# nurturenature/jepsen-tigerbeetle

Hardware: AMD Instinct MI355X
Metric: histories/sec, 10k-op/64-proc cas-register histories (time-to-verdict ms in extra) (higher is better)
Workload: dtype u64

## Files before the change

jepsen-tigerbeetle_amd/csrc/batch_create.hip:

```cpp
#include "tbc_batch.h"
#include "reach_table.h"

using namespace tbc;

namespace tbc {

uint64_t open_list_entries(const tbc_ops& c, uint64_t op_off, uint64_t n, uint32_t n_events, uint32_t n_slots,
                                  std::vector<uint32_t>& pre, bool branch_lists) {
  const uint64_t worst = std::max<uint64_t>(n, 1) * std::max(1u, n_slots);
  if (n == 0) return 1;
  if ((uint64_t)n_events > 64 * n + 1024) return worst;
  const uint32_t* inv = c.inv_pos + op_off;
  const uint32_t* ret = c.ret_pos + op_off;
  pre.assign((size_t)n_events + 1, 0u);
  for (uint64_t i = 0; i < n; i++) {
    if (ret[i] == TBC_POS_CRASHED) continue;
    if (ret[i] >= n_events || inv[i] > ret[i]) return worst;
    pre[ret[i] + 1] = 1;
  }
  for (uint32_t x = 1; x <= n_events; x++) pre[x] += pre[x - 1];
  uint64_t total = 0;
  const uint8_t* f = c.f + op_off;
  for (uint64_t i = 0; i < n; i++)
    if (ret[i] != TBC_POS_CRASHED && !(branch_lists && f[i] == TBC_F_READ)) total += pre[ret[i]] - pre[inv[i]] + 1;
// ... 327 lines not shown
    H.rec_off = tot.rec_n; tot.rec_n += n + 2ull * H.n_slots;
    H.seg_off = tot.seg_n; tot.seg_n += H.n_slots + 1;
    H.ret_off = H.op_off;
    H.bm_off = tot.bm_n; tot.bm_n += H.n_events / 32 + 1;
    H.frame_off = tot.frame_n; tot.frame_n += std::max<uint64_t>(n, 1) * B->frame_words;
    const uint64_t per_op = B->opts.visited_per_op ? B->opts.visited_per_op : 64;
    uint32_t lg = std::max(10u, ceil_log2(per_op * std::max<uint64_t>(n, 1)));
    while (lg > 10 && (1ull << lg) * KW * 8 > max_bytes) lg--;
    H.tab_log2 = lg;
    H.tab_off = tot.tab_n;
    if (!beam) { tot.tab_n += (1ull << lg) * KW; tot.tab_n = (tot.tab_n + 1) & ~1ull; }
    if (beam) {
      BeamHist& Q = bh[h];
      std::memset(&Q, 0, sizeof Q);
      uint32_t blg = lg;
      while (blg > 10 && ((1ull << blg) * EW * 8 > max_bytes || blg > kBeamMaxTabLog2)) blg--;
      Q.tab_log2 = blg;
      Q.off_off = tot.boff_n; tot.boff_n += n + 2;
      if (B->count_form) {
        const CountHist& ch = (*count_hist)[h];
        Q.cmem_off = tot.bocc_n; tot.bocc_n += ch.words.size();
        Q.n_classes = ch.n_classes; Q.top[0] = ch.top[0]; Q.top[1] = ch.top[1];
      }
      Q.lst_cap = lists_on_device ? 0xFFFFFFF0u : list_caps[h];
      Q.lst_off = tot.blst_n; tot.blst_n += lists_on_device ? 0u : Q.lst_cap;
      Q.stack_off = tot.bstack_n; tot.bstack_n += (1ull << blg);
      Q.tab_off = tot.btab_n; tot.btab_n += (1ull << blg);
    }
  }
  if (B->sweep) { tot.bstack_n = 0; tot.btab_n = 0; }
  return TBC_OK;
}

}

void tbc_batch::count_device_bytes() {
  tbc_batch* const B = this;
  const bool beam = B->width > 1;
  B->device_bytes = B->d_f.bytes() + B->d_a.bytes() + B->d_b.bytes() + B->d_proc.bytes() + B->d_inv.bytes() +
                    B->d_ret.bytes() + B->d_hist.bytes() + B->d_rec.bytes() + B->d_seg.bytes() + B->d_ret_slot.bytes() +
                    B->d_ret_op.bytes() + B->d_bitmap.bytes() + B->d_wpre.bytes() + B->d_frames.bytes() +
                    B->d_tab.bytes() + B->d_results.bytes() + B->d_work.bytes() + B->d_witness.bytes();
  if (beam) B->device_bytes += B->d_bh.bytes() + B->d_off.bytes() + B->d_ncr.bytes() + B->d_lst.bytes() +
                               B->d_crashed.bytes() + B->d_slot8.bytes() + B->d_rk8.bytes() + B->d_twn.bytes() + B->d_rdm.bytes() + B->d_look.bytes() + B->d_looktmp.bytes() + B->d_dstack.bytes() + B->d_stack.bytes() + B->d_btab.bytes() + B->d_pool.bytes() + B->d_cmem.bytes();
  if (B->d_stage[0].p) B->device_bytes += B->d_stage[0].bytes();
  if (B->d_stage[1].p) B->device_bytes += B->d_stage[1].bytes();
}

tbc_batch::~tbc_batch() {
  tbc::stream_release(this);
  d_f.release(); d_a.release(); d_b.release(); d_proc.release(); d_inv.release(); d_ret.release();
  d_hist.release(); d_rec.release(); d_seg.release(); d_ret_slot.release(); d_ret_op.release();
  d_bitmap.release(); d_wpre.release(); d_frames.release(); d_witness.release(); d_work.release();
  d_queue.release(); d_tab.release(); d_results.release(); d_table.release(); d_pool_vals.release(); d_cfg.release();
  d_bh.release(); d_off.release(); d_ncr.release(); d_lst.release(); d_crashed.release(); d_stack.release();
  d_zncr.release(); d_reach.release(); d_reach_hdr.release(); d_abort.release(); d_order.release(); d_park.release();
  if (abort_one) (void)hipHostFree(abort_one);
  if (progress) (void)hipHostFree(progress);
  d_progress.release();
  if (!borrowed) { for (auto& e : ev2) if (e) (void)hipEventDestroy(e); if (stream2) (void)hipStreamDestroy(stream2); }
  d_cmem.release(); d_occ.release(); d_btab.release(); d_slot8.release(); d_rk8.release(); d_look.release(); d_looktmp.release(); d_twn.release(); d_rdm.release(); d_cuts.release(); d_seglist.release(); d_sres.release(); d_dstack.release(); d_pool.release(); d_pool_cursor.release();
  if (ev_turn) (void)hipEventDestroy(ev_turn);
  if (!borrowed) {
    for (auto& e : ev) if (e) (void)hipEventDestroy(e);
    if (stream) (void)hipStreamDestroy(stream);
  }
}

namespace tbc {
namespace {

tbc_status alloc_arenas(CreatePlan& P) {
  tbc_batch* B = P.B; const tbc_opts* opts = P.opts; const tbc_model* model = P.model;
  const uint32_t nh = P.nh;
  const bool beam = P.beam, device_sizing = P.device_sizing;
  const LayoutTotals& t = P.tot;
  const uint32_t EW = B->entry_words();
  tbc_status s;
  const uint64_t T = B->total_ops;
  if (!t_ctx) {
    HIP_TRY(hipHostMalloc((void**)&B->progress, 16 * sizeof(uint32_t), hipHostMallocMapped | hipHostMallocCoherent));
    std::memset(B->progress, 0, 16 * sizeof(uint32_t));
    if ((s = B->d_progress.alloc(1))) return s;
  }
  if ((s = B->d_f.alloc(T)) || (s = B->d_a.alloc(T)) || (s = B->d_b.alloc(T)) || (s = B->d_proc.alloc(T)) ||
      (s = B->d_inv.alloc(T)) || (s = B->d_ret.alloc(T)) || (s = B->d_hist.alloc(nh)) || (s = B->d_bh.alloc(beam ? nh : 0)) || (s = B->d_work.alloc(nh)) ||
      (s = B->d_bitmap.alloc(t.bm_n)) || (s = B->d_off.alloc(beam ? t.boff_n : 0)) || (s = B->d_ncr.alloc(beam ? t.boff_n : 0)) || (s = B->d_pool_cursor.alloc(1)) ||
      (s = B->d_rec.alloc(t.rec_n)) ||
      (s = B->d_seg.alloc(t.seg_n)) || (s = B->d_ret_slot.alloc(T)) || (s = B->d_ret_op.alloc(T)) ||
      (s = B->d_wpre.alloc(t.bm_n)) || (s = B->d_frames.alloc(t.frame_n)) ||
      (s = B->d_tab.alloc(t.tab_n)) || (s = B->d_results.alloc(nh)) ||
      (s = B->d_queue.alloc(4)) || (s = B->d_witness.alloc(opts->want_witness ? T : 0)))
    return s;
  if (beam) {
    if ((!device_sizing && (s = B->d_lst.alloc(t.blst_n))) || (s = B->d_crashed.alloc((B->count_form || !B->any_crashed) ? 0 : T)) || (s = B->d_cmem.alloc(B->count_form ? t.bocc_n : 0)) ||
        (s = B->d_slot8.alloc(slot8_bytes(T, nh))) || (s = B->d_stack.alloc(t.bstack_n)) || (s = B->d_btab.alloc(t.btab_n * B->tab_stride())))
      return s;
    if ((B->sweep || B->rsweep) && ((s = B->d_cuts.alloc((uint64_t)nh * B->max_segs)) || (s = B->d_sres.alloc((uint64_t)nh * B->max_segs * kSweepSlices)) || (s = B->d_seglist.alloc((uint64_t)nh * B->max_segs * kSweepSlices * 3)))) return s;
    if (B->sweep || B->rsweep) B->seg_host.resize((size_t)nh * B->max_segs * kSweepSlices);
    if (B->rsweep) {
      std::vector<uint32_t> reach, hdr;
      for (uint32_t h = 0; h < nh; h++) {
        const CountHist& ch = B->count_hist[h];
        hdr.push_back((uint32_t)reach.size());
        hdr.push_back(build_reach_table(ch.words.data(), ch.n_classes, reach));
      }
      if ((s = B->d_zncr.alloc(t.boff_n)) || (s = B->d_reach.alloc(reach.size())) || (s = B->d_reach_hdr.alloc(hdr.size())) || (s = B->d_abort.alloc(nh))) return s;
      HIP_TRY(hipMemset(B->d_zncr.p, 0, B->d_zncr.bytes()));
      HIP_TRY(hipMemcpy(B->d_reach.p, reach.data(), reach.size() * 4, hipMemcpyHostToDevice));
      HIP_TRY(hipMemcpy(B->d_reach_hdr.p, hdr.data(), hdr.size() * 4, hipMemcpyHostToDevice));
      HIP_TRY(hipHostMalloc((void**)&B->abort_one, sizeof(uint32_t), hipHostMallocDefault));
      *B->abort_one = 1u;
    }
    if (B->lanes && (s = B->d_rk8.alloc(slot8_bytes(T, nh)))) return s;
    if (B->reg_rules() && ((!device_sizing && (s = B->d_twn.alloc(t.blst_n * B->mask_words))) || (s = B->d_rdm.alloc(B->lanes ? 1 : T * B->vpad * B->mask_words)))) return s;
    if (B->lanes) { B->d_rdm.release(); if ((s = B->d_rdm.alloc(T * B->front_words()))) return s; }
    const bool by_front = B->mask_words == 1 && B->vpad <= 32;
    if (B->lookahead && ((s = B->d_look.alloc(look_words(T, nh, B->mask_words))) || (s = B->d_looktmp.alloc(by_front ? 0 : T)) ||
                         (s = B->d_dstack.alloc(t.bstack_n)))) return s;
    {
      uint64_t biggest = 0;
      for (uint32_t h = 0; h < nh; h++) biggest = std::max<uint64_t>(biggest, 1ull << B->bh[h].tab_log2);
      uint64_t words = std::max<uint64_t>(t.btab_n * B->tab_stride() * (B->lanes ? 1u : 3u) / 10, biggest * (4 + 16 + 4) * (EW + 1));
      words = std::min<uint64_t>(words, (32ull << 30) / 8);
      if (B->sweep) words = 1;
      if ((s = B->d_pool.alloc(words))) return s;
    }
  }
  if ((s = B->d_cfg.alloc((uint64_t)nh * kCfgCap * (2 + B->mask_words)))) return s;
  if (beam && (s = B->d_park.alloc((uint64_t)nh * kParkWords))) return s;
  B->pool_len = P.desc->cols.pool ? P.desc->cols.pool_len : 0;
  if ((s = B->d_pool_vals.alloc(B->pool_len))) return s;
  if (B->pool_len) HIP_TRY(hipMemcpy(B->d_pool_vals.p, P.desc->cols.pool, (size_t)B->pool_len * 4, hipMemcpyHostToDevice));
  if (model->kind == TBC_MODEL_TABLE) {
    const size_t tn = (size_t)model->n_states * model->n_classes;
    B->table_host.assign(model->table, model->table + tn);
    if ((s = B->d_table.alloc(tn))) return s;
    HIP_TRY(hipMemcpy(B->d_table.p, B->table_host.data(), tn * 2, hipMemcpyHostToDevice));
    B->model.table = nullptr;
  }
  B->count_device_bytes();
  return TBC_OK;
}

tbc_status take_streams(tbc_batch* B) {
  if (t_ctx) {
    B->borrowed = true; B->stream = t_ctx->stream;
    for (int i = 0; i < 6; i++) B->ev[i] = t_ctx->ev[i];
    if (B->rsweep) {
      if (!t_ctx->stream2) {
        HIP_TRY(hipStreamCreateWithFlags(&t_ctx->stream2, hipStreamNonBlocking));
        for (auto& e : t_ctx->ev2) HIP_TRY(hipEventCreate(&e));
      }
      B->stream2 = t_ctx->stream2; B->ev2[0] = t_ctx->ev2[0]; B->ev2[1] = t_ctx->ev2[1];
    }
  } else {
    HIP_TRY(hipStreamCreateWithFlags(&B->stream, hipStreamNonBlocking));
    for (auto& e : B->ev) HIP_TRY(hipEventCreate(&e));
    if (B->rsweep) {
      HIP_TRY(hipStreamCreateWithFlags(&B->stream2, hipStreamNonBlocking));
      for (auto& e : B->ev2) HIP_TRY(hipEventCreate(&e));
    }
  }
  return TBC_OK;
}

tbc_status upload_inputs(CreatePlan& P, bool* done) {
  tbc_batch* B = P.B; const tbc_batch_desc* desc = P.desc;
  const uint32_t nh = P.nh;
  const bool beam = P.beam, device_sizing = P.device_sizing;
  const uint64_t T = B->total_ops, bocc_n = P.tot.bocc_n;
  *done = false;
  std::vector<uint32_t> work(nh);
  for (uint32_t h = 0; h < nh; h++) work[h] = h;
  if (t_ctx && T && !(B->count_form && bocc_n) && !device_sizing) {
    char* const base = (char*)B->d_f.p;
    const auto at = [&](const void* p) { return (size_t)((const char*)p - base); };
    const auto a256 = [](size_t b) { return (b + 255) & ~(size_t)255; };
    const bool consecutive = !B->d_f.owned && !B->d_a.owned && !B->d_b.owned && !B->d_proc.owned && !B->d_inv.owned && !B->d_ret.owned && !B->d_hist.owned &&
                             !B->d_bh.owned && !B->d_work.owned && at(B->d_a.p) == a256(T) && at(B->d_b.p) == at(B->d_a.p) + a256(T * 4) &&
                             at(B->d_proc.p) == at(B->d_b.p) + a256(T * 4) && at(B->d_inv.p) == at(B->d_proc.p) + a256(T * 4) && at(B->d_ret.p) == at(B->d_inv.p) + a256(T * 4) &&
                             at(B->d_hist.p) == at(B->d_ret.p) + a256(T * 4) && at(B->d_bh.p) == at(B->d_hist.p) + a256(nh * sizeof(Hist)) &&
                             at(B->d_work.p) == at(B->d_bh.p) + a256(std::max<size_t>(beam ? nh : 0, 1) * sizeof(BeamHist));
    if (consecutive) {
      const size_t total = at(B->d_work.p) + a256((size_t)nh * 4);
      B->upload_stage.resize(total);
      if (B->upload_stage.own.empty()) {
        char* st = B->upload_stage.data();
        std::memcpy(st, desc->cols.f, T);
        std::memcpy(st + at(B->d_a.p), desc->cols.a, T * 4);
        std::memcpy(st + at(B->d_b.p), desc->cols.b, T * 4);
        std::memcpy(st + at(B->d_proc.p), B->count_form ? P.slot_col.data() : desc->cols.process, T * 4);
        std::memcpy(st + at(B->d_inv.p), desc->cols.inv_pos, T * 4);
        std::memcpy(st + at(B->d_ret.p), desc->cols.ret_pos, T * 4);
        std::memcpy(st + at(B->d_hist.p), B->hist.data(), nh * sizeof(Hist));
        if (beam) std::memcpy(st + at(B->d_bh.p), B->bh.data(), nh * sizeof(BeamHist));
        std::memcpy(st + at(B->d_work.p), work.data(), (size_t)nh * 4);
        HIP_TRY(hipMemcpyAsync(base, st, total, hipMemcpyHostToDevice, B->stream));
        B->inputs_fresh = true;
        *done = true;
        TRACE("create: inputs queued as one block");
        return TBC_OK;
      }
    }
  }
  if (T) {
    HIP_TRY(hipMemcpyAsync(B->d_f.p, desc->cols.f, T, hipMemcpyHostToDevice, B->stream));
    HIP_TRY(hipMemcpyAsync(B->d_a.p, desc->cols.a, T * 4, hipMemcpyHostToDevice, B->stream));
    HIP_TRY(hipMemcpyAsync(B->d_b.p, desc->cols.b, T * 4, hipMemcpyHostToDevice, B->stream));
    HIP_TRY(hipMemcpyAsync(B->d_proc.p, B->count_form ? P.slot_col.data() : desc->cols.process, T * 4, hipMemcpyHostToDevice, B->stream));
    HIP_TRY(hipMemcpyAsync(B->d_inv.p, desc->cols.inv_pos, T * 4, hipMemcpyHostToDevice, B->stream));
    HIP_TRY(hipMemcpyAsync(B->d_ret.p, desc->cols.ret_pos, T * 4, hipMemcpyHostToDevice, B->stream));
  }
  std::vector<uint64_t> cmem_host;
  if (B->count_form && bocc_n) {
    cmem_host.reserve(bocc_n);
    for (uint32_t h = 0; h < nh; h++) cmem_host.insert(cmem_host.end(), B->count_hist[h].words.begin(), B->count_hist[h].words.end());
    HIP_TRY(hipMemcpyAsync(B->d_cmem.p, cmem_host.data(), cmem_host.size() * 8, hipMemcpyHostToDevice, B->stream));
  }
  HIP_TRY(hipMemcpyAsync(B->d_hist.p, B->hist.data(), nh * sizeof(Hist), hipMemcpyHostToDevice, B->stream));
  HIP_TRY(hipMemcpyAsync(B->d_work.p, work.data(), nh * 4, hipMemcpyHostToDevice, B->stream));
  HIP_TRY(hipStreamSynchronize(B->stream));
  TRACE("create: inputs resident");
  return TBC_OK;
}
// ... 157 lines not shown
```

jepsen-tigerbeetle_amd/csrc/batch_run.hip:

```cpp
#include "tbc_batch.h"
#include "witness_expand.h"

using namespace tbc;

namespace tbc {

static SearchArgs make_search_args(tbc_batch* B, uint64_t* tab, uint32_t n_work) {
  SearchArgs a{};
  a.hist = B->d_hist.p; a.rec = B->d_rec.p; a.seg = B->d_seg.p; a.ret_slot = B->d_ret_slot.p;
  a.ret_op = B->d_ret_op.p;
  a.frames = B->d_frames.p; a.tab = tab; a.results = B->d_results.p;
  a.witness = B->opts.want_witness ? B->d_witness.p : nullptr;
  a.work = B->d_work.p; a.queue = B->d_queue.p;
  a.table = B->d_table.p; a.n_work = n_work; a.model_kind = B->model.kind;
  a.init_state = B->model.init;
  a.n_classes = B->model.n_classes; a.n_states = B->model.n_states;
  a.max_steps = B->opts.max_steps;
  a.time_limit_ticks = B->opts.time_limit_ms * 100000ull;
  a.dbg = debug_words();
  a.pool_vals = B->d_pool_vals.p;
  a.cfg = B->d_cfg.p;
  a.progress = B->progress; a.progress_dev = B->d_progress.p;
  return a;
}

PackArgs make_pack_args(tbc_batch* B) {
  PackArgs pa{};
  pa.hist = B->d_hist.p; pa.f = B->d_f.p; pa.a = B->d_a.p; pa.b = B->d_b.p; pa.process = B->d_proc.p;
  pa.inv_pos = B->d_inv.p; pa.ret_pos = B->d_ret.p; pa.rec = B->d_rec.p; pa.seg = B->d_seg.p;
  pa.ret_slot = B->d_ret_slot.p; pa.ret_op = B->d_ret_op.p; pa.bitmap = B->d_bitmap.p; pa.wpre = B->d_wpre.p;
  pa.scratch = B->d_frames.p; pa.frame_words = B->frame_words; pa.n_hist = B->n_hist;
  pa.model_kind = B->model.kind; pa.n_classes = B->model.n_classes; pa.dbg = debug_words();
  pa.pool_vals = B->d_pool_vals.p; pa.pool_len = B->pool_len; pa.n_keys = B->model.n_keys;
  return pa;
}

PackOpenArgs make_pack_open_args(tbc_batch* B) {
  PackOpenArgs po{};
  po.hist = B->d_hist.p; po.bh = B->d_bh.p; po.f = B->d_f.p; po.a = B->d_a.p; po.b = B->d_b.p; po.process = B->d_proc.p;
  po.scratch = B->d_frames.p; po.off = B->d_off.p; po.ncr = B->d_ncr.p; po.lst = B->d_lst.p;
  po.rec = B->d_rec.p; po.seg = B->d_seg.p; po.chunks_per_hist = (uint32_t)((B->max_ops + 63) / 64);
  po.crashed = B->d_crashed.p; po.ret_slot = B->d_ret_slot.p; po.slot8 = B->d_slot8.p;
  po.ret_op = B->d_ret_op.p; po.look = B->lookahead ? B->d_look.p : nullptr; po.tmp = B->d_looktmp.p; po.n_hist = B->n_hist; po.mask_words = B->mask_words;
  po.branch_lists = (B->rules & kRuleBranch) ? 1u : 0u;
  po.rk8 = B->lanes ? B->d_rk8.p : nullptr; po.front_words = B->front_words(); po.front_compact = B->front_words() == kFrontCompactWords ? 1u : 0u;
  po.twn = B->reg_rules() ? B->d_twn.p : nullptr; po.rdm = (B->reg_rules() || B->lanes) ? B->d_rdm.p : nullptr; po.vpad = B->vpad;
  po.cmem = B->count_form ? B->d_cmem.p : nullptr;
  po.list_order = B->list_order();
  po.order_of = (!B->hist_order.empty() && B->d_order.p) ? B->d_order.p : nullptr;
  return po;
}

static uint32_t search_blocks(uint32_t n_work) {
  return std::max(1u, (n_work + kWavesPerBlock - 1) / kWavesPerBlock);
}

static BeamArgs make_beam_args(tbc_batch* B, uint64_t* tab, uint32_t* stack, uint32_t* dstack, uint32_t n_work) {
  BeamArgs a{};
  a.hist = B->d_hist.p; a.bh = B->d_bh.p; a.off = B->d_off.p; a.ncr = B->d_ncr.p; a.lst = B->d_lst.p;
  a.crashed = B->d_crashed.p; a.slot8 = B->d_slot8.p; a.look = B->lookahead ? B->d_look.p : nullptr; a.ret_slot = B->d_ret_slot.p; a.ret_op = B->d_ret_op.p;
  a.stack = stack; a.dstack = B->lookahead ? dstack : nullptr; a.tab = tab; a.results = B->d_results.p;
  a.witness = B->opts.want_witness ? B->d_witness.p : nullptr;
  a.work = B->d_work.p; a.table = B->d_table.p; a.n_work = n_work; a.model_kind = B->model.kind;
  const bool comm = B->model.kind == TBC_MODEL_SET || B->model.kind == TBC_MODEL_BANK;
  a.init_state = comm ? 0 : B->model.init;
  a.model_aux = B->model.init; a.n_keys = B->model.n_keys;
  a.n_classes = B->model.n_classes; a.width = B->width;
  a.round_budget = B->opts.round_budget;
  a.cmem = B->d_cmem.p; a.count_mode = kCountExact; a.tab_stride = B->entry_words(); a.epoch = 0;
  a.rules = B->rules; a.twn = B->d_twn.p; a.rdm = B->d_rdm.p; a.vpad = B->vpad; a.rk8 = B->d_rk8.p; a.front_words = B->front_words(); a.next_work = B->d_queue.p;
  a.max_steps = B->opts.max_steps;
  a.time_limit_ticks = B->opts.time_limit_ms * 100000ull;
  a.dbg = debug_words();
  a.pool_vals = B->d_pool_vals.p;
  a.cfg = B->d_cfg.p;
  a.pool = B->d_pool.p; a.pool_cursor = B->d_pool_cursor.p; a.pool_words = B->d_pool.n;
  a.abort = B->ext_abort; a.abort_set = B->ext_abort_set; a.abort_map = B->ext_abort_map;
  a.park = B->d_park.p; a.resume = 0;
  a.progress = B->progress; a.progress_dev = B->d_progress.p;
  {
    const uint64_t max_bytes = B->opts.max_visited_bytes ? B->opts.max_visited_bytes : (1ull << 30);
    uint32_t lg = 10;
    while (lg < kBeamMaxTabLog2 && (1ull << (lg + 1)) * B->entry_words() * 8 <= max_bytes) lg++;
    a.max_tab_log2 = lg;
  }
  return a;
}

static tbc_status scratch_pass(tbc_batch* B, const std::vector<uint32_t>& grp, const std::vector<uint32_t>& lg,
                               bool beam, const HostBuf<Hist>& hist_back, const HostBuf<BeamHist>& bh_back,
                               uint32_t width_override = 0, uint32_t count_mode = kCountExact, const std::vector<uint32_t>* targets = nullptr,
                               int64_t steps_override = -1) {
  hipStream_t s = B->stream;
  const uint32_t KW = 1 + B->mask_words, EW = B->entry_words();
  const uint64_t words_per_entry = beam ? EW : KW;
  uint64_t entries = 0;
  std::vector<Hist> ph(grp.size());
  std::vector<BeamHist> pb(beam ? grp.size() : 0);
  for (size_t i = 0; i < grp.size(); i++) {
    ph[i] = hist_back[grp[i]];
    if (beam) {
      pb[i] = bh_back[grp[i]];
// ... 1104 lines not shown
```

jepsen-tigerbeetle_amd/csrc/open_walk_impl.h:

```cpp
#pragma once
#include "wave_env.h"
#include "tbc_internal.h"

namespace tbc {
namespace walk {

constexpr uint32_t kCandCap = 136;
constexpr uint32_t kCandWords = 8;
constexpr uint32_t kAuxWords = 80;
constexpr uint32_t kKeyWords = 32, kKeyBits = 32 * kKeyWords;
static_assert(2 * kKeyWords <= kAuxWords && kKeyWords == 32, "the map and its prefix fit the scratch; two rows of 16 lanes scan it");
constexpr uint32_t kCursorWords = 64 + 32;
WV_HD constexpr uint32_t walk_lds_words() { return kCandCap * kCandWords + kAuxWords + kCursorWords; }
static_assert(4u * walk_lds_words() * sizeof(uint32_t) <= 20u * 1024u, "eight blocks of four wavefronts a CU");
constexpr uint32_t kTogWords = 64 * 4, kRankCntWords = 24;
constexpr uint32_t kSparseCand = kCandCap - (kTogWords + kRankCntWords) / kCandWords;
constexpr int kSparseSets = 2;
static_assert(kSparseCand <= 64u * kSparseSets, "two sets of 64 candidates");
static_assert((kTogWords + kRankCntWords) % kCandWords == 0u && (kSparseCand * kCandWords) % 4u == 0u && kSparseCand >= 96u, "the toggle words of a front are 16 bytes, aligned");
#ifndef TBC_WALK_BLOCKS
#define TBC_WALK_BLOCKS 8
#endif

constexpr uint32_t kCList = 1u;
// ... 541 lines not shown
    look[(uint64_t)F * 2u] = w0;
    look[(uint64_t)F * 2u + 1u] = pm;
  }
  }

  uint64_t w6 = 0ull, w7 = 0ull;
  if (compact) {
    if (by_ret) wv::barrier();
    aux[lane] = active ? rank_code(px, xf, xa, V) : (7u << 6);
    if (lane < kFrontCompactRanks - 1u) {
      const uint32_t G = F_lo + 64u + lane;
      uint32_t code = 7u << 6;
      if (G < R) {
        const uint32_t gx = A.ret_op[H->ret_off + G];
        code = rank_code(A.ret_slot[H->ret_off + G], A.f[H->op_off + gx], A.a[H->op_off + gx], V);
      }
      aux[64u + lane] = code;
    }
    wv::barrier();
    WV_UNROLL
    for (uint32_t l = 0; l < kFrontCompactRanks; l++) w7 |= (uint64_t)aux[lane + l] << (9u * l);
    const uint32_t nl = pos - pos0, nc = A.ncr[B->off_off + Fc];
    w6 = (uint64_t)pos0 | ((uint64_t)(nl & 0xFFu) << 32) | ((uint64_t)((nl + nc) & 0xFFFFFFu) << 40);
  }
  if (active && rdm && compact) {
    uint64_t* row = rdm + (uint64_t)F * FW;
    row[6] = w6; row[7] = w7;
  }
  return F_lo + 64u < R;
}

template <int VCAP>
WV_DEV void walk_wave(const PackOpenArgs& A, uint32_t wid, uint32_t* lds, uint32_t lane) {
  const uint32_t cph = A.chunks_per_hist;
  const uint32_t hr = wid / cph, c = wid - hr * cph, h = A.h0 + hr;
  if (h >= A.n_hist) return;
  (void)walk_chunk<VCAP>(A, h, c, lds, lane, false);
}

WV_HD constexpr uint32_t walk_runs_per_hist(uint32_t chunks_per_hist, uint32_t run = kWalkRun) { return (chunks_per_hist + run - 1u) / run; }

template <int VCAP, uint32_t RUN = kWalkRun>
WV_DEV void walk_run(const PackOpenArgs& A, uint32_t run_id, uint32_t* lds, uint32_t lane) {
  const uint32_t rph = walk_runs_per_hist(A.chunks_per_hist, RUN);
  const uint32_t hr = run_id / rph, c0 = (run_id - hr * rph) * RUN, h = A.h0 + hr;
  if (h >= A.n_hist) return;
  WV_NOUNROLL
  for (uint32_t j = 0; j < RUN; j++) {
    if (!walk_chunk<VCAP>(A, opaque_uniform(h), c0 + j, lds, wv::opaque(lane), j != 0u)) break;
    wv::barrier();
  }
}

}
}
```

jepsen-tigerbeetle_amd/csrc/pack_open.hip:

```cpp
#include <hip/hip_runtime.h>
#include <cstdlib>
#include <cstring>
#include "tbc_internal.h"
#include "open_walk_impl.h"

namespace tbc {

namespace {

__device__ __forceinline__ uint32_t ld_agent(const uint32_t* p) {
  return __hip_atomic_load(p, __ATOMIC_RELAXED, __HIP_MEMORY_SCOPE_AGENT);
}
__device__ __forceinline__ uint64_t ld_agent64(const uint64_t* p) {
  return __hip_atomic_load(p, __ATOMIC_RELAXED, __HIP_MEMORY_SCOPE_AGENT);
}

__device__ __forceinline__ void scan_parts(uint32_t* part, uint32_t NT, uint32_t* total_slot) {
  if (threadIdx.x < 64) {
    const uint32_t lane = threadIdx.x, per = NT / 64, lo = lane * per;
    uint32_t sum = 0;
    for (uint32_t i = 0; i < per; i++) sum += part[lo + i];
    uint32_t x = sum;
    for (uint32_t d = 1; d < 64; d <<= 1) { const uint32_t y = __shfl_up(x, d); if (lane >= d) x += y; }
    uint32_t run = x - sum;
    for (uint32_t i = 0; i < per; i++) { const uint32_t v = part[lo + i]; part[lo + i] = run; run += v; }
    if (lane == 63 && total_slot) *total_slot = x;
  }
}

constexpr uint32_t kBatch = 8;
template <class F>
__device__ __forceinline__ void chunk_loads(const uint32_t* p, uint32_t lo, uint32_t hi, F&& each) {
  for (uint32_t i = lo; i < hi; i += kBatch) {
    uint32_t v[kBatch];
#pragma unroll
    for (uint32_t k = 0; k < kBatch; k++) v[k] = i + k < hi ? ld_agent(&p[i + k]) : 0u;
#pragma unroll
    for (uint32_t k = 0; k < kBatch; k++) if (i + k < hi) each(i + k, v[k]);
  }
}

}

__global__ __launch_bounds__(1024) void open_counts_kernel(PackOpenArgs A) {
  __shared__ uint32_t s_part[1024];
  const uint32_t NT = blockDim.x;
  __shared__ uint32_t s_total;
  const uint32_t tid = threadIdx.x;
  const uint32_t MW = A.mask_words;

  for (uint32_t h = A.h0 + blockIdx.x; h < A.n_hist; h += gridDim.x) {
    const Hist* H = &A.hist[h];
    BeamHist* B = &A.bh[h];
    const uint32_t n = H->n_ops, R = H->n_ret;
    if (H->status != 0 || R == 0) {
// ... 292 lines not shown
          const uint32_t vi = rdm_index(va, V);
          if (lane == vi && (vi != 0u || va == TBC_NIL)) mine[j] |= 1ull << l;
        }
      }
      if (lane < V) {
#pragma unroll
        for (int j = 0; j < MW; j++) rdm[(uint64_t)F * FW + lane * MW + j] = mine[j];
      }
    }
    if (look) {
      const uint32_t jx = px >> 6, lx = px & 63u;
      uint32_t xf = kFNone, xinv = 0; int32_t xa = 0, xb = 0;
#pragma unroll
      for (int j = 0; j < MW; j++) if (jx == (uint32_t)j) {
        xf = __builtin_amdgcn_readlane(cur[j].f, lx); xinv = __builtin_amdgcn_readlane(cur[j].inv, lx);
        xa = (int32_t)__builtin_amdgcn_readlane((uint32_t)cur[j].a, lx); xb = (int32_t)__builtin_amdgcn_readlane((uint32_t)cur[j].b, lx);
      }
      const uint32_t need = look_need(xf, xa), prod = look_prod(xf, xa, xb), di = min(F - xinv, 255u);
      const uint64_t w0 = (uint64_t)(px & 0xFFFFu) | (uint64_t)need << 16 | (uint64_t)prod << 24 | (uint64_t)di << 32 | (255ull << 40);
      const uint32_t LW = 1 + MW;
#pragma unroll
      for (int j = 0; j < MW; j++) {
        const bool other = (live[j] || crashed_open[j]) && !(jx == (uint32_t)j && lane == lx);
        const uint64_t pm = need == kLookNone ? 0ull : __ballot(other && cur[j].prod == need);
        if (lane == 0) look[(uint64_t)F * LW + 1 + j] = pm;
      }
      if (lane == 0) { look[(uint64_t)F * LW] = w0; tmp[F] = 255u; }
    }
#pragma unroll
    for (int j = 0; j < MW; j++) {
      if (twn) {
#pragma unroll
        for (int w = 0; w < MW; w++) if ((px >> 6) == (uint32_t)w) tw[j][w] &= ~(1ull << (px & 63u));
      }
      if ((px >> 6) == (uint32_t)j && lane == (px & 63u)) {
        if (twn) {
#pragma unroll
          for (int w = 0; w < MW; w++) tw[j][w] = 0ull;
          known[j] = false;
        }
        cur[j] = nxt[j];
        at[j] = min(at[j] + 1u, tail[j]);
        nxt[j] = load_cur(rec + min(at[j] + 1u, tail[j]));
      }
    }
  }
}

template <int VCAP>
__global__ __launch_bounds__(256, VCAP <= 8 ? TBC_WALK_BLOCKS : 2) void open_walk_fronts_kernel(PackOpenArgs A) {
  extern __shared__ __attribute__((aligned(16))) uint32_t walk_lds[];
  const uint32_t lane = threadIdx.x & 63u;
  const uint32_t wv_ = (uint32_t)__builtin_amdgcn_readfirstlane((int)(threadIdx.x >> 6));
  walk::walk_run<VCAP>(A, blockIdx.x * 4u + wv_, walk_lds + wv_ * walk::walk_lds_words(), lane);
}

__global__ __launch_bounds__(1024) void open_dprod_kernel(PackOpenArgs A) {
  const uint32_t NT = blockDim.x, tid = threadIdx.x, MW = A.mask_words;
  for (uint32_t h = A.h0 + blockIdx.x; h < A.n_hist; h += gridDim.x) {
    const Hist* H = &A.hist[h];
    const BeamHist* B = &A.bh[h];
    const uint32_t n = H->n_ops, R = H->n_ret;
    if (H->status != 0 || B->status != 0 || R == 0) continue;
    const uint8_t* f = A.f + H->op_off;
    const int32_t* a = A.a + H->op_off;
    const int32_t* b = A.b + H->op_off;
    const uint32_t* sc_inv = A.scratch + H->frame_off;
    const uint32_t* sc_ret = sc_inv + n;
    const uint32_t LW = 1 + MW;
    uint64_t* look = A.look + look_off(H->op_off, h, MW);
    const uint32_t* ret_op = A.ret_op + H->ret_off;
    uint32_t* tmp = A.tmp + H->op_off;
    for (uint32_t i = tid; i < n; i += NT) {
      const uint32_t pv = look_prod(f[i], a[i], b[i]);
      if (pv == kLookNone || (sc_ret[i] == kInf && f[i] == TBC_F_READ)) continue;
      const uint32_t ir = sc_inv[i];
      uint64_t w[kLookahead]; uint32_t ro[kLookahead];
#pragma unroll
      for (uint32_t k = 0; k < kLookahead; k++) {
        const uint32_t t = ir + k;
        const bool in = t < R;
        w[k] = in ? ld_agent64(&look[(uint64_t)t * LW]) : 0ull;
        ro[k] = in ? ret_op[t] : 0u;
      }
#pragma unroll
      for (uint32_t k = 0; k < kLookahead; k++) {
        const uint32_t t = ir + k;
        if (t < R && ((uint32_t)(w[k] >> 16) & 0xFFu) == pv && ro[k] != i) atomicMin(&tmp[t], k);
      }
    }
    __syncthreads();
    for (uint32_t t0 = tid; t0 < R; t0 += 4u * NT) {
      uint32_t d[4]; uint64_t w0[4];
#pragma unroll
      for (uint32_t k = 0; k < 4; k++) {
        const uint32_t t = t0 + k * NT;
        d[k] = t < R ? ld_agent(&tmp[t]) : 255u;
        w0[k] = t < R ? ld_agent64(&look[(uint64_t)t * LW]) : 0ull;
      }
#pragma unroll
      for (uint32_t k = 0; k < 4; k++) {
        const uint32_t t = t0 + k * NT;
        if (t < R && d[k] < 255u) look[(uint64_t)t * LW] = (w0[k] & ~(255ull << 40)) | ((uint64_t)d[k] << 40);
      }
    }
    __syncthreads();
  }
// ... 30 lines not shown
  const uint32_t cph = A.chunks_per_hist * 64u;
  const uint64_t gid = (uint64_t)blockIdx.x * 256u + threadIdx.x;
  const uint32_t hr = (uint32_t)(gid / cph), F = (uint32_t)(gid - (uint64_t)hr * cph), h = A.h0 + hr;
  if (h >= A.n_hist) return;
  const Hist* H = &A.hist[h];
  const BeamHist* B = &A.bh[h];
  if (H->status != 0 || B->status != 0 || F >= H->n_ret) return;
  const uint32_t* off = A.off + B->off_off;
  const uint32_t o0 = off[F], o1 = off[F + 1u], nc = A.ncr[B->off_off + F];
  const uint8_t* s8 = A.slot8 + slot8_off(H->op_off, h) + F;
  const uint8_t* k8 = A.rk8 + slot8_off(H->op_off, h) + F;
  uint64_t w[4] = {0, 0, 0, 0};
#pragma unroll
  for (uint32_t l = 0; l < 16; l++) {
    w[l >> 3] |= (uint64_t)s8[l] << (8u * (l & 7u));
    w[2 + (l >> 3)] |= (uint64_t)k8[l] << (8u * (l & 7u));
  }
  if (A.front_compact) {
    uint64_t* rec = A.rdm + (H->op_off + F) * kFrontCompactWords;
    uint64_t win = 0;
#pragma unroll
    for (uint32_t l = 0; l < kFrontCompactRanks; l++) {
      const uint32_t sl = (uint32_t)(w[0] >> (8u * l)) & 63u, k = (uint32_t)(w[2] >> (8u * l)) & 0xFFu;
      win |= (uint64_t)(sl | ((k == 0xFFu ? 7u : (k & 7u)) << 6)) << (9u * l);
    }
    rec[6] = (uint64_t)o0 | ((uint64_t)((o1 - o0) & 0xFFu) << 32) | ((uint64_t)(((o1 - o0) + nc) & 0xFFFFFFu) << 40);
    rec[7] = win;
    return;
  }
  uint64_t* rec = A.rdm + (H->op_off + F) * A.front_words + A.vpad * A.mask_words;
  rec[0] = (uint64_t)o0 | ((uint64_t)(o1 - o0) << 32);
  rec[1] = (uint64_t)((o1 - o0) + nc);
  rec[2] = w[0]; rec[3] = w[1]; rec[4] = w[2]; rec[5] = w[3];
}

void launch_open_counts(const PackOpenArgs& a, void* stream) {
  const uint32_t n_here = a.n_hist - a.h0;
  hipLaunchKernelGGL(open_counts_kernel, dim3(n_here < 4096 ? n_here : 4096), dim3(n_here <= 64 ? 1024 : 256), 0, (hipStream_t)stream, a);
}

void launch_pack_open(const PackOpenArgs& a, void* stream, bool skip_counts) {
  hipStream_t s = (hipStream_t)stream;
  const uint32_t n_here = a.n_hist - a.h0;
  const uint32_t grid = n_here < 4096 ? n_here : 4096;
  const uint32_t nt = n_here <= 64 ? 1024 : 256;
  if (!skip_counts) hipLaunchKernelGGL(open_counts_kernel, dim3(grid), dim3(nt), 0, s, a);
  if (a.cmem) hipLaunchKernelGGL(count_fronts_kernel, dim3(grid), dim3(256), 0, s, a, 0u);
  const uint64_t waves = (uint64_t)n_here * a.chunks_per_hist;
  const uint32_t wgrid = (uint32_t)((waves + 3) / 4);
  const bool by_front = a.mask_words == 1 && a.vpad <= 32;
  const size_t walk_lds_bytes = 4u * walk::walk_lds_words() * sizeof(uint32_t);
  if (by_front) {
    const uint64_t runs = (uint64_t)n_here * walk::walk_runs_per_hist(a.chunks_per_hist);
    const uint32_t rgrid = (uint32_t)((runs + 3) / 4);
    if (a.vpad <= 8) hipLaunchKernelGGL(open_walk_fronts_kernel<8>, dim3(rgrid), dim3(256), walk_lds_bytes, s, a);
    else hipLaunchKernelGGL(open_walk_fronts_kernel<32>, dim3(rgrid), dim3(256), walk_lds_bytes, s, a);
  } else switch (a.mask_words) {
    case 2: hipLaunchKernelGGL(open_walk_kernel<2>, dim3(wgrid), dim3(256), 0, s, a); break;
    default: hipLaunchKernelGGL(open_walk_kernel<4>, dim3(wgrid), dim3(256), 0, s, a); break;
  }
  if (a.look && !by_front) hipLaunchKernelGGL(open_dprod_kernel, dim3(grid), dim3(nt), 0, s, a);
  if (a.cmem) hipLaunchKernelGGL(count_fronts_kernel, dim3(grid), dim3(256), 0, s, a, 1u);
  if (a.front_words && !(by_front && a.front_compact)) {
    const uint64_t fronts = (uint64_t)n_here * a.chunks_per_hist * 64u;
    hipLaunchKernelGGL(front_meta_kernel, dim3((uint32_t)((fronts + 255) / 256)), dim3(256), 0, s, a);
  }
}

}
```

jepsen-tigerbeetle_amd/csrc/tbc_batch.h:

```cpp
#pragma once
#include <hip/hip_runtime.h>
#include <algorithm>
#include <atomic>
#include <chrono>
#include <cstdio>
#include <cstdlib>
#include <cstring>
#include <deque>
#include <mutex>
#include <new>
#include <thread>
#include <vector>
#include "tbc_internal.h"
#include "pool_plan.h"

namespace tbc {

#define HIP_TRY(expr)                                                             \
  do {                                                                            \
    hipError_t e_ = (expr);                                                       \
    if (e_ != hipSuccess) {                                                       \
      ::tbc::set_error("%s failed: %s (%s:%d)", #expr, hipGetErrorString(e_), __FILE__, __LINE__); \
      return e_ == hipErrorOutOfMemory ? TBC_ERR_OOM : TBC_ERR_HIP;               \
    }                                                                             \
// ... 94 lines not shown
  T& operator[](size_t i) { return p[i]; }
  const T& operator[](size_t i) const { return p[i]; }
  T* begin() { return p; }
  T* end() { return p + n; }
  const T* begin() const { return p; }
  const T* end() const { return p + n; }
};

struct CountHist {
  std::vector<uint64_t> words;
  uint32_t n_classes = 0, n_slots = 1;
  uint64_t top[kCountWords] = {0, 0};
};

struct LayoutTotals {
  uint64_t rec_n = 0, seg_n = 0, bm_n = 0, frame_n = 0, tab_n = 0;
  uint64_t boff_n = 0, bocc_n = 0, blst_n = 0, bstack_n = 0, btab_n = 0;
  uint64_t max_ops = 1, total_ops = 0;
};

}

struct tbc_pending_input {
  uint32_t stage = 0;
  uint32_t slot = 0;
  uint32_t n_hist = 0;
  uint64_t total_ops = 0, max_ops = 1;
  std::vector<tbc::Hist> hist;
  std::vector<tbc::BeamHist> bh;
  tbc::LayoutTotals tot;
  std::vector<tbc::CountHist> count_hist;
  std::vector<uint64_t> cmem;
  uint64_t lst_total = 0;
};

struct tbc_batch {
  int device = 0;
  hipStream_t stream = nullptr;
  hipEvent_t ev[6] = {};
  uint32_t n_hist = 0;
  uint64_t total_ops = 0, max_ops = 1;
  uint32_t mask_words = 1;
  uint32_t frame_words = 6;
  tbc_model model{};
  tbc_opts opts{};
  std::vector<tbc::Hist> hist;
  std::vector<uint16_t> table_host;
  tbc::DevBuf<uint8_t> d_f;
  tbc::DevBuf<int32_t> d_a, d_b, d_proc;
  tbc::DevBuf<uint32_t> d_inv, d_ret;
  tbc::DevBuf<tbc::Hist> d_hist;
  tbc::DevBuf<tbc::Rec> d_rec;
  tbc::DevBuf<uint32_t> d_seg, d_ret_slot, d_ret_op, d_bitmap, d_wpre, d_frames, d_witness, d_work, d_queue;
  tbc::DevBuf<uint64_t> d_tab;
  tbc::DevBuf<tbc::DevResult> d_results;
  tbc::DevBuf<uint16_t> d_table;
  tbc::DevBuf<int32_t> d_pool_vals;
  uint32_t pool_len = 0;
  tbc::DevBuf<uint64_t> d_cfg;
  uint32_t width = 1;
  uint32_t front_words() const { return !lanes ? 0u : ((rules & tbc::kRuleEager) && tbc::front_compact_ok(n_dom, mask_words)) ? tbc::kFrontCompactWords : tbc::front_stride(vpad, mask_words); }
  uint32_t lanes = 0;
  static constexpr uint32_t kDefaultListOrder = 16u + 24u;
  bool list_order_applies() const {
    return width > 1 && mask_words == 1 && vpad <= 32 && !(rules & tbc::kRuleCount) && !sweep && opts.round_budget == 0 &&
           (model.kind == TBC_MODEL_REGISTER || model.kind == TBC_MODEL_CAS_REGISTER);
  }
  uint32_t list_order() const {
    if (order_override != kNoOrderOverride) return order_override;
    if (!list_order_applies() || opts.list_order == TBC_ORDER_SLOT) return 0u;
    if (opts.list_order == TBC_ORDER_DEFAULT) return kDefaultListOrder;
    return opts.list_order >= 16u ? opts.list_order : opts.list_order - 1u;
  }
  static constexpr uint32_t kNoOrderOverride = 0xFFFFFFFFu;
  uint32_t order_override = kNoOrderOverride;
  std::vector<uint32_t> order_of_hist;
  const uint32_t* ext_abort = nullptr;
  uint32_t* ext_abort_set = nullptr;
  const uint32_t* ext_abort_map = nullptr;
  std::vector<uint32_t> hist_order;
  tbc::DevBuf<uint32_t> d_order;
  tbc::DevBuf<uint32_t> d_park;
  uint32_t last_raced = 0;
  uint32_t* progress = nullptr;
  tbc::DevBuf<uint32_t> d_progress;
  mutable std::atomic<uint32_t> progress_seen{0};
  std::atomic<uint64_t> run_t0{0};
  std::atomic<uint32_t> running{0};
  bool order_restarts_apply() const {
    return width > 1 && !lanes && !count_form && list_order_applies() && opts.list_order == TBC_ORDER_DEFAULT && opts.max_steps == 0 &&
           !(opts.dominance & TBC_DOM_NO_ORDER_RESTARTS);
  }
  std::vector<tbc::BeamHist> bh;
  tbc::DevBuf<tbc::BeamHist> d_bh;
  tbc::DevBuf<uint32_t> d_off, d_ncr, d_stack;
  tbc::DevBuf<tbc::OpRec> d_lst, d_crashed;
  tbc::DevBuf<uint8_t> d_slot8;
  tbc::DevBuf<uint8_t> d_rk8;
  bool lookahead = false;
  tbc::DevBuf<uint64_t> d_look;
  tbc::DevBuf<uint32_t> d_dstack;
  tbc::DevBuf<uint32_t> d_looktmp;
  bool sweep = false;
  uint32_t max_segs = 1, seg_target = 0, cut_open = 0, n_dom = 1;
  tbc::DevBuf<uint32_t> d_cuts, d_seglist;
  tbc::DevBuf<tbc::SegResult> d_sres;
// ... 86 lines not shown
```

jepsen-tigerbeetle_amd/csrc/tbc_internal.h:

```cpp
#pragma once
#include <cstdarg>
#include <cstdint>
#include "../../include/tbcheck.h"

namespace tbc {

void set_error(const char* fmt, ...);

constexpr uint32_t kInf = 0xFFFFFFFFu;
constexpr uint32_t kMaxSlots = 1024;
constexpr uint32_t kWavesPerBlock = 4;
constexpr uint32_t kBlock = 64 * kWavesPerBlock;
constexpr uint8_t kFNone = 0xFF;
constexpr uint32_t kBeamMaxTabLog2 = 28;
constexpr uint32_t kCfgCap = 256;

struct __attribute__((aligned(16))) Rec {
  uint32_t inv_rank;
  uint32_t ret_rank;
  uint32_t opidx;
  uint32_t f;
  int32_t a, b;
  uint32_t cls;
  uint32_t prod;
// ... 136 lines not shown
  return (v == TBC_NIL || (uint32_t)(v + 1) >= vpad) ? 0u : (uint32_t)(v + 1);
}

struct __attribute__((aligned(16))) BeamHist {
  uint64_t off_off;
  uint64_t cmem_off;
  uint64_t lst_off;
  uint64_t stack_off;
  uint64_t tab_off;
  uint32_t lst_cap;
  uint32_t tab_log2;
  uint32_t n_crashed;
  uint32_t status;
  uint32_t n_classes;
  uint32_t target;
  uint64_t top[kCountWords];
  uint32_t lst_need;
  uint32_t pad2[3];
};

struct PackOpenArgs {
  const Hist* hist;
  BeamHist* bh;
  const uint8_t* f;
  const int32_t* a;
  const int32_t* b;
  const int32_t* process;
  const uint32_t* scratch;
  const Rec* rec;
  const uint32_t* seg;
  uint32_t chunks_per_hist;
  uint32_t branch_lists;
  uint32_t* off;
  uint32_t* ncr;
  OpRec* lst;
  OpRec* crashed;
  const uint32_t* ret_slot;
  const uint32_t* ret_op;
  uint64_t* look;
  uint32_t* tmp;
  uint8_t* slot8;
  uint32_t front_words;
  uint32_t front_compact;
  uint8_t* rk8;
  uint32_t n_hist;
  uint32_t mask_words;
  uint64_t* twn;
  uint64_t* rdm;
  uint32_t vpad;
  uint32_t h0;
  const uint64_t* cmem;
  const uint32_t* order_of;
  uint32_t list_order;
};

__host__ __device__ inline uint64_t slot8_off(uint64_t op_off, uint64_t h) { return (op_off + 24ull * h) & ~7ull; }
__host__ __device__ inline uint64_t slot8_bytes(uint64_t total_ops, uint64_t n_hist) { return total_ops + 24ull * n_hist + 32ull; }

struct BeamArgs {
  const Hist* hist;
  const BeamHist* bh;
  const uint32_t* off;
  const uint32_t* ncr;
  const OpRec* lst;
  const OpRec* crashed;
  const uint64_t* look;
  const uint8_t* slot8;
  const uint32_t* ret_slot;
  const uint32_t* ret_op;
  uint32_t* stack;
  uint32_t* dstack;
  uint64_t* tab;
  DevResult* results;
  uint32_t* witness;
  const uint32_t* work;
  const uint16_t* table;
  uint32_t n_work;
  uint32_t model_kind;
  int32_t init_state;
  uint32_t n_classes;
  uint32_t width;
  uint32_t pad;
  uint64_t max_steps;
  uint64_t time_limit_ticks;
  uint32_t* dbg;
  uint32_t stall_checks;
  uint32_t pad_stall;
  const uint32_t* abort;
  uint64_t* pool;
  unsigned long long* pool_cursor;
  uint64_t pool_words;
  uint32_t max_tab_log2;
  uint32_t pad2;
  const int32_t* pool_vals;
  uint64_t* cfg;
  int32_t model_aux;
  uint32_t round_budget;
  uint32_t n_keys;
  uint32_t rules;
  const uint64_t* twn;
  const uint64_t* rdm;
  uint32_t vpad;
  uint32_t pad3;
  const uint8_t* rk8;
  uint32_t front_words;
  const uint64_t* cmem;
// ... 80 lines not shown
```

Before: 421,300.

## Replace static front-walk grid with persistent waves drawing runs from atomic queue

The front-walk kernel now launches only as many blocks as can stay resident (a configurable share of occupancy times CU count). Each wave repeatedly claims a run index from a global atomic counter instead of getting one fixed run from its block index. This is meant to balance uneven run lengths across waves and to cut block launch overhead. The cost is an atomic per run, a per-batch memset and a self-resetting counter protocol, and throughput drops if fewer resident waves leave the GPU underfilled.

```diff
diff --git a/jepsen-tigerbeetle_amd/csrc/batch_create.hip b/jepsen-tigerbeetle_amd/csrc/batch_create.hip
--- a/jepsen-tigerbeetle_amd/csrc/batch_create.hip
+++ b/jepsen-tigerbeetle_amd/csrc/batch_create.hip
@@ -403,7 +403,7 @@
   d_f.release(); d_a.release(); d_b.release(); d_proc.release(); d_inv.release(); d_ret.release();
   d_hist.release(); d_rec.release(); d_seg.release(); d_ret_slot.release(); d_ret_op.release();
   d_bitmap.release(); d_wpre.release(); d_frames.release(); d_witness.release(); d_work.release();
-  d_queue.release(); d_tab.release(); d_results.release(); d_table.release(); d_pool_vals.release(); d_cfg.release();
+  d_queue.release(); d_walk_queue.release(); d_tab.release(); d_results.release(); d_table.release(); d_pool_vals.release(); d_cfg.release();
   d_bh.release(); d_off.release(); d_ncr.release(); d_lst.release(); d_crashed.release(); d_stack.release();
   d_zncr.release(); d_reach.release(); d_reach_hdr.release(); d_abort.release(); d_order.release(); d_park.release();
   if (abort_one) (void)hipHostFree(abort_one);
@@ -441,7 +441,7 @@
       (s = B->d_seg.alloc(t.seg_n)) || (s = B->d_ret_slot.alloc(T)) || (s = B->d_ret_op.alloc(T)) ||
       (s = B->d_wpre.alloc(t.bm_n)) || (s = B->d_frames.alloc(t.frame_n)) ||
       (s = B->d_tab.alloc(t.tab_n)) || (s = B->d_results.alloc(nh)) ||
-      (s = B->d_queue.alloc(4)) || (s = B->d_witness.alloc(opts->want_witness ? T : 0)))
+      (s = B->d_queue.alloc(4)) || (s = B->d_walk_queue.alloc(2)) || (s = B->d_witness.alloc(opts->want_witness ? T : 0)))
     return s;
   if (beam) {
     if ((!device_sizing && (s = B->d_lst.alloc(t.blst_n))) || (s = B->d_crashed.alloc((B->count_form || !B->any_crashed) ? 0 : T)) || (s = B->d_cmem.alloc(B->count_form ? t.bocc_n : 0)) ||
@@ -522,6 +522,7 @@
   const bool beam = P.beam, device_sizing = P.device_sizing;
   const uint64_t T = B->total_ops, bocc_n = P.tot.bocc_n;
   *done = false;
+  HIP_TRY(hipMemsetAsync(B->d_walk_queue.p, 0, B->d_walk_queue.bytes(), B->stream));
   std::vector<uint32_t> work(nh);
   for (uint32_t h = 0; h < nh; h++) work[h] = h;
   if (t_ctx && T && !(B->count_form && bocc_n) && !device_sizing) {
diff --git a/jepsen-tigerbeetle_amd/csrc/batch_run.hip b/jepsen-tigerbeetle_amd/csrc/batch_run.hip
--- a/jepsen-tigerbeetle_amd/csrc/batch_run.hip
+++ b/jepsen-tigerbeetle_amd/csrc/batch_run.hip
@@ -48,6 +48,7 @@
   po.cmem = B->count_form ? B->d_cmem.p : nullptr;
   po.list_order = B->list_order();
   po.order_of = (!B->hist_order.empty() && B->d_order.p) ? B->d_order.p : nullptr;
+  po.walk_queue = B->d_walk_queue.p;
   return po;
 }
 
diff --git a/jepsen-tigerbeetle_amd/csrc/open_walk_impl.h b/jepsen-tigerbeetle_amd/csrc/open_walk_impl.h
--- a/jepsen-tigerbeetle_amd/csrc/open_walk_impl.h
+++ b/jepsen-tigerbeetle_amd/csrc/open_walk_impl.h
@@ -617,5 +617,51 @@
   }
 }
 
-}
-}
+constexpr uint32_t kStatWalkDraw = 54, kStatWalkDrawPast = 55;
+#if defined(TBC_EMU)
+inline void (*&emu_on_draw())(uint32_t) { static void (*f)(uint32_t) = nullptr; return f; }
+#endif
+#if !defined(TBC_EMU) && defined(TBC_WALK_QUEUE_CARRY)
+#error "the planted mutations of the front walk are for tests/emu (TBC_EMU) only"
+#endif
+template <int VCAP, uint32_t RUN = kWalkRun>
+WV_DEV void walk_queue(const PackOpenArgs& A, uint32_t* lds, uint32_t lane) {
+  uint32_t h = 0, c = 0, j = RUN;
+#if defined(TBC_WALK_QUEUE_CARRY)
+  bool had_run = false;
+#endif
+  WV_NOUNROLL
+  for (;;) {
+    if (j == RUN) {
+      const auto& C = *wv::cold(A);
+      const uint32_t rph = walk_runs_per_hist(C.chunks_per_hist, RUN), end = (C.n_hist - C.h0) * rph;
+      uint32_t t = 0;
+      if (lane == 0u) t = atomicAdd(&C.walk_queue[0], 1u);
+      const uint32_t run_id = wv::readlane(t, 0u);
+      if (run_id >= end) break;
+#if defined(TBC_EMU)
+      if (lane == 0u) { wv::stat(kStatWalkDraw, 1); if (emu_on_draw()) emu_on_draw()(run_id); }
+#endif
+      const uint32_t hr = run_id / rph;
+      h = C.h0 + hr; c = (run_id - hr * rph) * RUN; j = 0u;
+      wv::barrier();
+    }
+#if defined(TBC_WALK_QUEUE_CARRY)
+    const bool carried = j != 0u || had_run;
+    had_run = true;
+#else
+    const bool carried = j != 0u;
+#endif
+    const bool more = walk_chunk<VCAP>(A, opaque_uniform(h), c + j, lds, wv::opaque(lane), carried);
+    j = more ? j + 1u : RUN;
+    wv::barrier();
+  }
+  if (lane == 0u) {
+    wv::stat(kStatWalkDrawPast, 1);
+    const auto& C = *wv::cold(A);
+    if (atomicAdd(&C.walk_queue[1], 1u) + 1u == C.walk_waves) { wv::st32((wv::gu32*)&C.walk_queue[0], 0u); wv::st32((wv::gu32*)&C.walk_queue[1], 0u); }
+  }
+}
+
+}
+}
diff --git a/jepsen-tigerbeetle_amd/csrc/pack_open.hip b/jepsen-tigerbeetle_amd/csrc/pack_open.hip
--- a/jepsen-tigerbeetle_amd/csrc/pack_open.hip
+++ b/jepsen-tigerbeetle_amd/csrc/pack_open.hip
@@ -1,6 +1,9 @@
 #include <hip/hip_runtime.h>
+#include <algorithm>
 #include <cstdlib>
 #include <cstring>
+#include <mutex>
+#include <vector>
 #include "tbc_internal.h"
 #include "open_walk_impl.h"
 
@@ -399,7 +402,28 @@
   extern __shared__ __attribute__((aligned(16))) uint32_t walk_lds[];
   const uint32_t lane = threadIdx.x & 63u;
   const uint32_t wv_ = (uint32_t)__builtin_amdgcn_readfirstlane((int)(threadIdx.x >> 6));
-  walk::walk_run<VCAP>(A, blockIdx.x * 4u + wv_, walk_lds + wv_ * walk::walk_lds_words(), lane);
+  walk::walk_queue<VCAP>(A, walk_lds + wv_ * walk::walk_lds_words(), lane);
+}
+
+#ifndef TBC_WALK_RESIDENT_EIGHTHS
+#define TBC_WALK_RESIDENT_EIGHTHS 5u
+#endif
+static_assert(TBC_WALK_RESIDENT_EIGHTHS >= 1u && TBC_WALK_RESIDENT_EIGHTHS <= 8u, "a share of what stays resident");
+template <int VCAP>
+static uint32_t walk_resident_blocks(size_t lds_bytes) {
+  static std::mutex mu;
+  static std::vector<uint32_t> known;
+  int dev = 0;
+  if (hipGetDevice(&dev) != hipSuccess || dev < 0) dev = 0;
+  std::lock_guard<std::mutex> g(mu);
+  if (known.size() <= (size_t)dev) known.resize((size_t)dev + 1, 0u);
+  if (known[dev] == 0u) {
+    int per_cu = 0, cus = 0;
+    if (hipOccupancyMaxActiveBlocksPerMultiprocessor(&per_cu, open_walk_fronts_kernel<VCAP>, 256, lds_bytes) != hipSuccess || per_cu < 1) per_cu = 1;
+    if (hipDeviceGetAttribute(&cus, hipDeviceAttributeMultiprocessorCount, dev) != hipSuccess || cus < 1) cus = 1;
+    known[dev] = (((uint32_t)per_cu * TBC_WALK_RESIDENT_EIGHTHS + 7u) / 8u) * (uint32_t)cus;
+  }
+  return known[dev];
 }
 
 __global__ __launch_bounds__(1024) void open_dprod_kernel(PackOpenArgs A) {
@@ -536,9 +560,12 @@
   const size_t walk_lds_bytes = 4u * walk::walk_lds_words() * sizeof(uint32_t);
   if (by_front) {
     const uint64_t runs = (uint64_t)n_here * walk::walk_runs_per_hist(a.chunks_per_hist);
-    const uint32_t rgrid = (uint32_t)((runs + 3) / 4);
-    if (a.vpad <= 8) hipLaunchKernelGGL(open_walk_fronts_kernel<8>, dim3(rgrid), dim3(256), walk_lds_bytes, s, a);
-    else hipLaunchKernelGGL(open_walk_fronts_kernel<32>, dim3(rgrid), dim3(256), walk_lds_bytes, s, a);
+    const uint32_t resident = a.vpad <= 8 ? walk_resident_blocks<8>(walk_lds_bytes) : walk_resident_blocks<32>(walk_lds_bytes);
+    const uint32_t rgrid = (uint32_t)std::max<uint64_t>(1u, std::min<uint64_t>((runs + 3) / 4, resident));
+    PackOpenArgs q = a;
+    q.walk_waves = rgrid * 4u;
+    if (a.vpad <= 8) hipLaunchKernelGGL(open_walk_fronts_kernel<8>, dim3(rgrid), dim3(256), walk_lds_bytes, s, q);
+    else hipLaunchKernelGGL(open_walk_fronts_kernel<32>, dim3(rgrid), dim3(256), walk_lds_bytes, s, q);
   } else switch (a.mask_words) {
     case 2: hipLaunchKernelGGL(open_walk_kernel<2>, dim3(wgrid), dim3(256), 0, s, a); break;
     default: hipLaunchKernelGGL(open_walk_kernel<4>, dim3(wgrid), dim3(256), 0, s, a); break;
diff --git a/jepsen-tigerbeetle_amd/csrc/tbc_batch.h b/jepsen-tigerbeetle_amd/csrc/tbc_batch.h
--- a/jepsen-tigerbeetle_amd/csrc/tbc_batch.h
+++ b/jepsen-tigerbeetle_amd/csrc/tbc_batch.h
@@ -170,6 +170,7 @@
   tbc::DevBuf<tbc::Hist> d_hist;
   tbc::DevBuf<tbc::Rec> d_rec;
   tbc::DevBuf<uint32_t> d_seg, d_ret_slot, d_ret_op, d_bitmap, d_wpre, d_frames, d_witness, d_work, d_queue;
+  tbc::DevBuf<uint32_t> d_walk_queue;
   tbc::DevBuf<uint64_t> d_tab;
   tbc::DevBuf<tbc::DevResult> d_results;
   tbc::DevBuf<uint16_t> d_table;
diff --git a/jepsen-tigerbeetle_amd/csrc/tbc_internal.h b/jepsen-tigerbeetle_amd/csrc/tbc_internal.h
--- a/jepsen-tigerbeetle_amd/csrc/tbc_internal.h
+++ b/jepsen-tigerbeetle_amd/csrc/tbc_internal.h
@@ -212,6 +212,8 @@
   const uint64_t* cmem;
   const uint32_t* order_of;
   uint32_t list_order;
+  uint32_t walk_waves;
+  uint32_t* walk_queue;
 };
 
 __host__ __device__ inline uint64_t slot8_off(uint64_t op_off, uint64_t h) { return (op_off + 24ull * h) & ~7ull; }
```

Result: no change. 421,200 (-0.0%).
